# lpiccinelli-eth/UniDepth

Hardware: AMD Instinct MI355X
Metric: images/sec (whole node) + p50 latency, ViT-L/14 518x518 bs=8 (higher is better)
Workload: dtype f16; 1 GPU; UniDepthV2 vitl14 infer(), 518x518, bs=8 per GPU, all 7 outputs on device; value = 2 independent infer() calls in flight per GPU (HIP streams); value_one_call / p50_latency_ms = one call at a time; global_batch=8, parallelism=dp1, inflight=2

## Files before the change

### unidepth_amd/csrc/gemm.hip

```cpp
#include "ud_common.h"

#ifdef UD_TRACE
__device__ unsigned long long* ud_trace_ptr = nullptr;
#define UD_STAMP(slot)                                                                           \
  do {                                                                                           \
    if (ud_trace_ptr && threadIdx.x == 0 && trace_tile < 8)                                      \
      ud_trace_ptr[((size_t)blockIdx.x * 8 + trace_tile) * 8 + (slot)] = wall_clock64();         \
  } while (0)
#else
#define UD_STAMP(slot)
#endif

namespace {

constexpr int UD_LNC_TILES = 2;
constexpr int UD_LNC_PLANE = UD_LNC_TILES * 256;

template <int BN_, int WM_, int WN_>
struct Cfg {
  static constexpr int BM = 128, BN = BN_, BK = 64, WM = WM_, WN = WN_;
  static constexpr int NWM = BM / WM, NWN = BN / WN;
  static constexpr int TM = WM / 16, TN = WN / 16;
  static constexpr int A_BYTES = BM * BK * 2;
  static constexpr int B_BYTES = BN * BK * 2;
// ... 561 lines not shown

template <class C, int EPI, int AMODE, int NST = 2, bool SPLIT = false>
__global__ __launch_bounds__(256) void gemm_kernel(const UdGemm p) {
  extern __shared__ __attribute__((aligned(16))) char smem[];
  const int tiles_n = (p.N + C::BN - 1) / C::BN;
  const int tiles_m = (p.M + C::BM - 1) / C::BM;
  const int nblk = tiles_m * tiles_n;
  int bid = blockIdx.x;
  if constexpr (SPLIT) {
    const int tile_m = (bid >> 1) / tiles_n, tile_n = (bid >> 1) - tile_m * tiles_n;
    gemm_body<C, EPI, AMODE, true, NST, true>(p, smem, tile_m * C::BM, tile_n * C::BN, (const half_t*)p.A, (const half_t*)p.W, p.bias,
                                              (char*)p.out, (char*)p.out2, p.w2, p.b2, p.post_add, bid >> 1, bid & 1);
    return;
  }
  {
    const int q = nblk >> 3, r = nblk & 7;
    const int xcd = bid & 7, idx = bid >> 3;
    bid = (xcd < r ? xcd * (q + 1) : r * (q + 1) + (xcd - r) * q) + idx;
  }
  const int tile_m = bid / tiles_n;
  const int tile_n = bid - tile_m * tiles_n;
  const int m0 = tile_m * C::BM, n0 = tile_n * C::BN;
  const int g = blockIdx.z;
  const half_t* A = (const half_t*)p.A + (long long)g * p.gA;
  const half_t* W = (const half_t*)p.W + (long long)g * p.gW;
  const float* bias = p.bias ? p.bias + (long long)g * p.gBias : nullptr;
  char* out = (char*)p.out + (long long)g * p.gOut * ((EPI == UD_EPI_F16 || EPI == UD_EPI_QKV) ? 2 : 4);
  char* out2 = p.out2 ? (char*)p.out2 + (long long)g * p.gOut2 * 2 : nullptr;
  const float* w2 = p.w2 ? p.w2 + (long long)g * p.gW2 : nullptr;
  const float b2 = g == 0 ? p.b2 : p.b2_g1;
  const float post_add = g == 0 ? p.post_add : p.post_add_g1;
  if constexpr (EPI == UD_EPI_QKV) {
    if (n0 >= p.vsplit) {
      gemm_body<C, EPI, AMODE, false, NST, false>(p, smem, m0, n0, A, W, bias, out, out2, w2, b2, post_add);
      return;
    }
  }
  gemm_body<C, EPI, AMODE, true, NST, false>(p, smem, m0, n0, A, W, bias, out, out2, w2, b2, post_add);
}

template <int MH>
struct BigCfg {
  static constexpr int BM = 64 * MH;
  static constexpr int A_BYTES = BM * 128;
  static constexpr int STAGE = A_BYTES + 32768;
  static constexpr int A_LOADS = BM / 64;
};

template <bool B> struct BoolTag { static constexpr bool value = B; };
constexpr int LNC_TILES = UD_LNC_TILES;
constexpr int LNC_LDS = 2 * UD_LNC_PLANE * 4;

__device__ __forceinline__ void ud_pair16(unsigned& a, unsigned& b) {
  const auto r = __builtin_amdgcn_permlane16_swap(a, b, false, false);
  a = r[0];
  b = r[1];
}
__device__ __forceinline__ void ud_pair32(unsigned& a, unsigned& b) {
  const auto r = __builtin_amdgcn_permlane32_swap(a, b, false, false);
  a = r[0];
  b = r[1];
}
__device__ __forceinline__ unsigned ud_pack2(float x, float y) {
  f32x2 v; v[0] = x; v[1] = y;
  const half2v h = __builtin_convertvector(v, half2v);
  return __builtin_bit_cast(unsigned, h);
}
typedef __attribute__((ext_vector_type(4))) unsigned u32x4;

template <int R, int M>
__device__ __forceinline__ void ud_interleave_reads() {
  constexpr int q = M / (R + 1);
  if constexpr (R >= 1) { __builtin_amdgcn_sched_group_barrier(0x8, q, 0); __builtin_amdgcn_sched_group_barrier(0x100, 1, 0); }
  if constexpr (R >= 2) { __builtin_amdgcn_sched_group_barrier(0x8, q, 0); __builtin_amdgcn_sched_group_barrier(0x100, 1, 0); }
  if constexpr (R >= 3) { __builtin_amdgcn_sched_group_barrier(0x8, q, 0); __builtin_amdgcn_sched_group_barrier(0x100, 1, 0); }
  if constexpr (R >= 4) { __builtin_amdgcn_sched_group_barrier(0x8, q, 0); __builtin_amdgcn_sched_group_barrier(0x100, 1, 0); }
  if constexpr (R >= 5) { __builtin_amdgcn_sched_group_barrier(0x8, q, 0); __builtin_amdgcn_sched_group_barrier(0x100, 1, 0); }
  if constexpr (R >= 6) { __builtin_amdgcn_sched_group_barrier(0x8, q, 0); __builtin_amdgcn_sched_group_barrier(0x100, 1, 0); }
  if constexpr (R >= 7) { __builtin_amdgcn_sched_group_barrier(0x8, q, 0); __builtin_amdgcn_sched_group_barrier(0x100, 1, 0); }
  if constexpr (R >= 8) { __builtin_amdgcn_sched_group_barrier(0x8, q, 0); __builtin_amdgcn_sched_group_barrier(0x100, 1, 0); }
  __builtin_amdgcn_sched_group_barrier(0x8, M - q * R, 0);
}

template <int MH, int EPI, int AMODE, bool BAL = false, bool LNC = false, bool GRP = false, bool W3 = false, bool SPK = false>
__global__ __launch_bounds__(512) void gemm256_kernel(const UdGemm p) {
  extern __shared__ __attribute__((aligned(16))) char smem[];
  using C = BigCfg<MH>;
  static_assert(!W3 || (AMODE == UD_A_DENSE && !BAL && !GRP), "W3: dense A, tile list");
  static_assert(!SPK || (!BAL && !LNC && !GRP && !W3 && (EPI == UD_EPI_F16 || EPI == UD_EPI_F32)), "K split: plain tile list, fp16 / fp32 epilogues");
  constexpr int RING_BYTES = W3 ? 2 * C::A_BYTES + 3 * 32768 : 2 * C::STAGE;
  static_assert(!LNC || (AMODE == UD_A_DENSE && (EPI == UD_EPI_F16 || EPI == UD_EPI_QKV)), "LayerNorm-folded consumer: dense A, fp16 outputs");
  constexpr int BM = C::BM;
  constexpr int TM = 2 * MH;
  const int tid = threadIdx.x;
  const int lane = tid & 63;
  const int wv = __builtin_amdgcn_readfirstlane(tid >> 6);
  const int wm = wv >> 2, wn = wv & 3;
  const int nk = SPK ? (p.K >> 7) : (p.K >> 6);
  const int kbase = SPK ? (int)(blockIdx.x & 1) * nk : 0;
  const int tiles_n = (p.N + 255) >> 8;
  const int tiles_m = (p.M + BM - 1) / BM;
  const int nblk = tiles_m * tiles_n;
  const half_t* A = (const half_t*)p.A;
  const half_t* W = (const half_t*)p.W;

  auto decode = [&](int t, int& m0, int& n0) {
    const int q = nblk >> 3, r = nblk & 7;
    const int xcd = t & 7, idx = t >> 3;
    const int bid = (xcd < r ? xcd * (q + 1) : r * (q + 1) + (xcd - r) * q) + idx;
    const int GM = nblk <= 256 ? 1 : 8;
    const int gsz = GM * tiles_n;
    const int grp = bid / gsz;
    const int first_m = grp * GM;
    const int gm = (tiles_m - first_m) < GM ? (tiles_m - first_m) : GM;
    const int rem = bid - grp * gsz;
    m0 = (first_m + rem % gm) * BM;
    n0 = (rem / gm) << 8;
  };

  const int lrow = tid >> 3;
  const int csrc = (tid & 7) ^ ((lrow >> 1) & 7);
  const ud_rsrc_t rA = ud_make_rsrc(A, 0x80000000u);
  const ud_rsrc_t rW = ud_make_rsrc(W, 0x80000000u);
  unsigned pa[C::A_LOADS];
  unsigned cyx[C::A_LOADS];
  unsigned pb[4];
  const float inv_cc = (AMODE != UD_A_DENSE) ? 1.0f / (float)(p.Cin >> 3) : 0.0f;
  auto setupA = [&](int m0, int mh) {
    int grp = 0;
    if constexpr (GRP) grp = m0 / p.grp_rows;
#pragma unroll
    for (int i = 0; i < C::A_LOADS; ++i) {
      if (i >= mh) continue;
      int m = m0 + lrow + 64 * i;
      m = m < p.M ? m : p.M - 1;
      if constexpr (GRP) {
        if (p.gA == 0) m -= grp * p.grp_rows;
      }
      if constexpr (AMODE == UD_A_DENSE) {
        pa[i] = ((unsigned)m * (unsigned)p.lda + csrc * 8) * 2u;
      } else {
        const int img = m / p.rows_img;
        const int pp = m - img * p.rows_img;
        const int y = pp / p.Wimg;
        pa[i] = (unsigned)((long long)img * p.img_stride) * 2u;
        cyx[i] = pp < p.Himg * p.Wimg ? ((unsigned)y << 16) | (unsigned)(pp - y * p.Wimg) : 0x40000000u;
      }
    }
  };
  auto setupB = [&](int m0, int n0) {
    int grp = 0;
    if constexpr (GRP) grp = m0 / p.grp_rows;
#pragma unroll
    for (int i = 0; i < 4; ++i) {
      int n = n0 + lrow + 64 * i;
      n = n < p.N ? n : p.N - 1;
      pb[i] = ((unsigned)n * (unsigned)p.ldw + csrc * 8) * 2u;
      if constexpr (GRP) pb[i] += (unsigned)grp * (unsigned)p.gW * 2u;
    }
  };
  auto setup = [&](int m0, int n0, int mh) {
    setupA(m0, mh);
    setupB(m0, n0);
  };
  const int a_wt = p.a_wrap > 0 ? (AMODE == UD_A_DENSE ? p.a_wrap >> 6 : p.a_wrap) : 0x7fffffff;
  const int w_wt = p.w_wrap > 0 ? p.w_wrap >> 6 : 0x7fffffff;
  auto a_stage = [&](int stg) -> char* { return smem + stg * (W3 ? C::A_BYTES : C::STAGE); };
  auto b_stage = [&](int stg) -> char* { return W3 ? smem + 2 * C::A_BYTES + stg * 32768 : smem + stg * C::STAGE + C::A_BYTES; };
  auto issueA = [&](int kt, int stg, int mh) {
    char* sb = a_stage(stg) + wv * 1024;
    kt += kbase;
// ... 14 lines not shown
      for (int i = 0; i < C::A_LOADS; ++i) {
        if (i >= mh) continue;
        const int yy = (int)(cyx[i] >> 16) + dy, xx = (int)(cyx[i] & 0xffff) + dx;
        const bool ok = tap < 9 && (unsigned)yy < (unsigned)p.Himg && (unsigned)xx < (unsigned)p.Wimg;
        const unsigned off = ok ? pa[i] + (unsigned)((yy * p.Wimg + xx) * p.cstride + p.coff + cch) * 2u : 0xfffffff0u;
        ud_bufl16(rA, off, 0, sb + i * 8192);
      }
    }
  };
  auto issueB = [&](int kt, int stg) {
    char* sb = b_stage(stg) + wv * 1024;
    kt += kbase;
    const int kb = kt >= w_wt ? kt - w_wt : kt;
#pragma unroll
    for (int i = 0; i < 4; ++i) ud_bufl16(rW, pb[i], kb * 128, sb + i * 8192);
  };
  auto issue = [&](int kt, int stg, int mh) {
    issueA(kt, stg, mh);
    issueB(kt, stg);
  };

  const int fswz = (lane & 15) >> 1;
  const int c0 = ((lane >> 4) ^ fswz) << 4;
  const int c1 = ((4 + (lane >> 4)) ^ fswz) << 4;
  const int b_off = (wn * 64 + (lane & 15)) * 128;

  f32x4 acc[TM][4];
  half8 a0[MH], a1[MH], b0[4], b1[4];
  int stg = 0;
  int stgb = 0;

  constexpr bool ACC_EPI = (EPI == UD_EPI_F32);

  float* const lds_rstd = (float*)(smem + RING_BYTES);
  float* const lds_nm = lds_rstd + UD_LNC_PLANE;
  int tl = 0;

  int m0, n0, mhc = MH;
  int t = SPK ? (int)(blockIdx.x >> 1) : (int)blockIdx.x;
  int bal_k = 0, bal_tb = 0, bal_te = 0, bal_u0 = 0, bal_n0 = 0;
  if constexpr (BAL) {
    const int G = gridDim.x;
    const int cpc = G / tiles_n;
    const int U = (p.M + 63) >> 6;
    int col, r;
    if ((G & 7) == 0 && (cpc & 3) == 0 && (tiles_n & 1) == 0) {
      const int x = blockIdx.x & 7, j = blockIdx.x >> 3;
      const int cx = tiles_n >> 1, rx = cpc >> 2;
      col = (x & 1) * cx + j % cx;
      r = (x >> 1) * rx + j / cx;
    } else if (tiles_n == 1 && (G & 7) == 0) {
      col = 0;
      r = (blockIdx.x & 7) * (G >> 3) + (blockIdx.x >> 3);
    } else {
      const int lc = blockIdx.x;
      col = lc / cpc;
      r = lc - col * cpc;
    }
    const int base = U / cpc, extra = U - base * cpc;
    const int un = base + (r < extra ? 1 : 0);
    if (un == 0) return;
    bal_u0 = r * base + (r < extra ? r : extra);
    bal_k = (un + 3) >> 2;
    bal_tb = un / bal_k;
    bal_te = un - bal_tb * bal_k;
    bal_n0 = col << 8;
    t = 0;
  }
  auto tile_at = [&](int i, int& tm0, int& tn0, int& tmh) {
    if constexpr (BAL) {
      tmh = bal_tb + (i < bal_te ? 1 : 0);
      tm0 = (bal_u0 + i * bal_tb + (i < bal_te ? i : bal_te)) << 6;
      tn0 = bal_n0;
    } else {
      decode(i, tm0, tn0);
      tmh = MH;
    }
  };
  const int tcount = BAL ? bal_k : nblk;
  const int tstep = BAL ? 1 : (SPK ? nblk : (int)gridDim.x);
  tile_at(t, m0, n0, mhc);
  setup(m0, n0, mhc);
  issue(0, 0, mhc);
  if constexpr (W3) issueB(1, 1);
  const ud_rsrc_t rS = ud_make_rsrc(LNC ? p.row_stats_in : nullptr, (unsigned)p.M * 8u);
  auto stats_dma = [&](int tm0, int tmh, int buf) {
    if (wv < 4 && wv < tmh) {
      int m = tm0 + wv * 64 + lane;
      m = m < p.M ? m : p.M - 1;
      ud_bufl4(rS, (unsigned)m * 8u, 0, lds_rstd + buf * 256 + wv * 64);
      ud_bufl4(rS, (unsigned)m * 8u + 4u, 0, lds_nm + buf * 256 + wv * 64);
    }
  };
  if constexpr (LNC) stats_dma(m0, mhc, 0);

  int trace_tile = 0;
  bool first = true;
  for (; t < tcount; t += tstep, ++trace_tile) {
    UD_STAMP(0);
    const int tn = t + tstep;
    const bool has_next = tn < tcount;
    int m0n = 0, n0n = 0, mhn = MH;
    if (has_next) tile_at(tn, m0n, n0n, mhn);
    const bool swap = !(EPI == UD_EPI_QKV && n0 >= p.vsplit);
    auto tile_body = [&](auto MHT) {
    constexpr int MHC = decltype(MHT)::value;
    constexpr int TMC = 2 * MHC;
    constexpr int BMC = 64 * MHC;
    const int a_off = (wm * (BMC / 2) + (lane & 15)) * 128;
    const int mbase = m0 + wm * (BMC / 2), nbase = n0 + wn * 64;

#pragma unroll
    for (int i = 0; i < TMC; ++i)
#pragma unroll
      for (int j = 0; j < 4; ++j) acc[i][j] = (f32x4){0.f, 0.f, 0.f, 0.f};

    bool counted = false;
    if constexpr (ACC_EPI) {
      if (p.accumulate && kbase == 0) {
        int ln = lane;
        asm volatile("" : "+v"(ln));
        if (first && (m0 + BMC <= p.M) && (n0 + 256 <= p.N) && p.rows_in == 0) {
          const float* ob = (const float*)p.out + (size_t)(mbase + (ln & 15)) * p.ldc + nbase + 4 * (ln >> 4);
#pragma unroll
          for (int i = 0; i < TMC; ++i)
#pragma unroll
            for (int j = 0; j < 4; ++j) acc[i][j] = *(const f32x4*)(ob + (size_t)(i * 16) * p.ldc + j * 16);
          counted = true;
        } else {
          gemm_preload_acc<TMC, 4>(p, acc, mbase, nbase, ln, (const char*)p.out);
        }
      }
    }
    if (first) {
      if (counted) asm volatile("s_waitcnt vmcnt(%0)" ::"i"(TMC * 4) : "memory");
      else asm volatile("s_waitcnt vmcnt(0)" ::: "memory");
      __builtin_amdgcn_s_barrier();
      asm volatile("" ::: "memory");
      first = false;
    }
    {
      const char* sa0 = a_stage(stg);
      const char* sb0 = b_stage(W3 ? stgb : stg);
#pragma unroll
      for (int i = 0; i < MHC; ++i) a0[i] = *(const half8*)(sa0 + a_off + i * 2048 + c0);
#pragma unroll
      for (int j = 0; j < 4; ++j) b0[j] = *(const half8*)(sb0 + b_off + j * 2048 + c0);
    }

    auto ktile = [&](auto SW, auto LASTT, int kt, auto PHT) {
      constexpr bool SWAP = decltype(SW)::value;
      constexpr bool LAST = decltype(LASTT)::value;
      constexpr int PH = decltype(PHT)::value;
      const int stgb1 = stgb == 2 ? 0 : stgb + 1, stgb2 = stgb == 0 ? 2 : stgb - 1;
      const char* sa = a_stage(stg);
      const char* sb = b_stage(W3 ? stgb : stg);
      const char* san = a_stage(stg ^ 1);
      const char* sbn = b_stage(W3 ? stgb1 : stg ^ 1);
#define UD_MFMA_HALF(ROW0, AF, BF)                                                                               \
  _Pragma("unroll") for (int i = 0; i < MHC; ++i) _Pragma("unroll") for (int j = 0; j < 4; ++j) {               \
    if constexpr (SWAP) acc[ROW0 + i][j] = __builtin_amdgcn_mfma_f32_16x16x32_f16(BF[j], AF[i], acc[ROW0 + i][j], 0, 0, 0); \
    else acc[ROW0 + i][j] = __builtin_amdgcn_mfma_f32_16x16x32_f16(AF[i], BF[j], acc[ROW0 + i][j], 0, 0, 0);   \
  }
      if constexpr (W3) {
        if constexpr (PH == 2) {
          if (has_next) {
            if constexpr (LNC) stats_dma(m0n, mhn, (tl + 1) & 1);
            setupA(m0n, mhn);
            issueA(0, stg ^ 1, mhn);
            issueB(1, stgb2);
          }
        } else if constexpr (PH == 1) {
          issueA(kt + 1, stg ^ 1, MHC);
          if (has_next) {
            setupB(m0n, n0n);
            issueB(0, stgb2);
          }
        } else {
          issueA(kt + 1, stg ^ 1, MHC);
          issueB(kt + 2, stgb2);
        }
      } else if constexpr (LAST) {
        if (has_next) {
          setup(m0n, n0n, mhn);
          issue(0, stg ^ 1, mhn);
          if constexpr (LNC) stats_dma(m0n, mhn, (tl + 1) & 1);
        }
      } else {
        issue(kt + 1, stg ^ 1, MHC);
      }
#pragma unroll
      for (int i = 0; i < MHC; ++i) a1[i] = *(const half8*)(sa + a_off + (MHC + i) * 2048 + c0);
      UD_MFMA_HALF(0, a0, b0)
      ud_interleave_reads<MHC, 4 * MHC>();
      __builtin_amdgcn_sched_barrier(0);
#pragma unroll
      for (int i = 0; i < MHC; ++i) a0[i] = *(const half8*)(sa + a_off + i * 2048 + c1);
#pragma unroll
      for (int j = 0; j < 4; ++j) b1[j] = *(const half8*)(sb + b_off + j * 2048 + c1);
      UD_MFMA_HALF(MHC, a1, b0)
      ud_interleave_reads<MHC + 4, 4 * MHC>();
      __builtin_amdgcn_sched_barrier(0);
#pragma unroll
      for (int i = 0; i < MHC; ++i) a1[i] = *(const half8*)(sa + a_off + (MHC + i) * 2048 + c1);
      UD_MFMA_HALF(0, a0, b1)
      ud_interleave_reads<MHC, 4 * MHC>();
      __builtin_amdgcn_sched_barrier(0);
      if constexpr (W3) {
        if (PH == 0 || has_next) asm volatile("s_waitcnt vmcnt(4)\n\ts_waitcnt lgkmcnt(0)" ::: "memory");
        else asm volatile("s_waitcnt vmcnt(0)\n\ts_waitcnt lgkmcnt(0)" ::: "memory");
      } else {
        asm volatile("s_waitcnt vmcnt(0)\n\ts_waitcnt lgkmcnt(0)" ::: "memory");
      }
      __builtin_amdgcn_s_barrier();
      asm volatile("" ::: "memory");
      if constexpr (!LAST) {
#pragma unroll
        for (int i = 0; i < MHC; ++i) a0[i] = *(const half8*)(san + a_off + i * 2048 + c0);
#pragma unroll
        for (int j = 0; j < 4; ++j) b0[j] = *(const half8*)(sbn + b_off + j * 2048 + c0);
      }
      UD_MFMA_HALF(MHC, a1, b1)
      if constexpr (!LAST) ud_interleave_reads<MHC + 4, 4 * MHC>();
      __builtin_amdgcn_sched_barrier(0);
#undef UD_MFMA_HALF
      stg ^= 1;
      if constexpr (W3) stgb = stgb1;
    };

    auto kloop = [&](auto SW) {
      if constexpr (W3) {
        for (int kt = 0; kt < nk - 2; ++kt) ktile(SW, BoolTag<false>{}, kt, IntTag<0>{});
        ktile(SW, BoolTag<false>{}, nk - 2, IntTag<1>{});
        ktile(SW, BoolTag<true>{}, nk - 1, IntTag<2>{});
      } else {
        for (int kt = 0; kt < nk - 1; ++kt) ktile(SW, BoolTag<false>{}, kt, IntTag<0>{});
        ktile(SW, BoolTag<true>{}, nk - 1, IntTag<0>{});
      }
    };
    UD_STAMP(1);
    if constexpr (EPI == UD_EPI_QKV) {
      if (swap) kloop(BoolTag<true>{});
      else kloop(BoolTag<false>{});
    } else {
      kloop(BoolTag<true>{});
    }
    UD_STAMP(2);
    if constexpr (SPK) {
      constexpr int NQ = TMC * 4;
      const int half = (int)(blockIdx.x & 1);
      f32x4* mine = (f32x4*)p.splitk_ws + ((size_t)(t * 2 + half) * 8 + wv) * (NQ * 64) + lane;
      const f32x4* other = (const f32x4*)p.splitk_ws + ((size_t)(t * 2 + (half ^ 1)) * 8 + wv) * (NQ * 64) + lane;
#pragma unroll
      for (int i = 0; i < TMC; ++i)
#pragma unroll
        for (int j = 0; j < 4; ++j) {
          const f32x4 v = acc[i][j];
          asm volatile("global_store_dwordx4 %0, %1, off sc0 sc1\n\ts_nop 2" ::"v"(mine + (i * 4 + j) * 64), "v"(v) : "memory");
        }
      asm volatile("s_waitcnt vmcnt(0)" ::: "memory");
      __builtin_amdgcn_s_barrier();
      unsigned* tk = (unsigned*)(smem + RING_BYTES);
      if (tid == 0) *tk = atomicAdd((unsigned*)p.splitk_cnt + t, 1u);
      asm volatile("s_waitcnt lgkmcnt(0)" ::: "memory");
      __builtin_amdgcn_s_barrier();
      const unsigned ticket = *tk;
      if ((ticket & 1u) == 0) return;
#pragma unroll
      for (int c = 0; c < NQ / 8; ++c) {
        f32x4 o[8];
#pragma unroll
        for (int q = 0; q < 8; ++q) asm volatile("global_load_dwordx4 %0, %1, off sc0 sc1" : "=v"(o[q]) : "v"(other + (c * 8 + q) * 64) : "memory");
        asm volatile("s_waitcnt vmcnt(0)" : "+v"(o[0]), "+v"(o[1]), "+v"(o[2]), "+v"(o[3]), "+v"(o[4]), "+v"(o[5]), "+v"(o[6]), "+v"(o[7])::"memory");
#pragma unroll
        for (int q = 0; q < 8; ++q) acc[(c * 8 + q) >> 2][(c * 8 + q) & 3] += o[q];
      }
    }
    const float* const lnst = LNC ? lds_rstd + (tl & 1) * 256 + wm * (BMC / 2) : nullptr;

    const float* biasp = p.bias;
    if constexpr (GRP) {
      if (p.bias) biasp = p.bias + (long long)(m0 / p.grp_rows) * p.gBias;
    }
    const bool full = (m0 + BMC <= p.M) && (n0 + 256 <= p.N) && p.rows_in == 0 && p.add == nullptr && p.bias != nullptr;
    bool fast = false;
    bool ticket_taken = false;
    unsigned ticket_val = 0;
    int eln = lane;
    asm volatile("" : "+v"(eln));
    const int frow = eln & 15, fq = eln >> 4;
    if constexpr (EPI == UD_EPI_F16 || EPI == UD_EPI_QKV) {
      if (swap) {
        fast = full && (p.ldc & 7) == 0;
        if (fast) {
          const int act = p.act;
          f32x4 bv[4], ws[4];
#pragma unroll
          for (int j = 0; j < 4; ++j) bv[j] = *(const f32x4*)(biasp + nbase + j * 16 + 4 * fq);
          if constexpr (LNC) {
#pragma unroll
            for (int j = 0; j < 4; ++j) ws[j] = *(const f32x4*)(p.wsum + nbase + j * 16 + 4 * fq);
          }
          half_t* o = (half_t*)p.out + (size_t)(mbase + frow) * p.ldc + nbase + 16 * (fq & 1) + 8 * (fq >> 1);
          auto body = [&](auto ACT) {
            constexpr int AC = decltype(ACT)::value;
#pragma unroll
            for (int i = 0; i < TMC; ++i) {
              unsigned w[4][2];
              float rs = 0.f, nmr = 0.f;
              if constexpr (LNC) {
                rs = lnst[i * 16 + frow];
                nmr = lnst[UD_LNC_PLANE + i * 16 + frow];
              }
#pragma unroll
// ... 541 lines not shown
        const int hy = hp / 18, hx = hp - hy * 18;
        int iy = cur.y0 - 1 + hy, ix = cur.x0 - 1 + hx;
        iy = iy < 0 ? -iy : (iy >= p.Himg ? 2 * p.Himg - 2 - iy : iy);
        ix = ix < 0 ? -ix : (ix >= p.Wimg ? 2 * p.Wimg - 2 - ix : ix);
        const bool ok = hp < 324 && iy >= cur.ylo && iy <= cur.yhi && ix >= cur.xlo && ix <= cur.xhi;
        half8 o8;
#pragma unroll
        for (int e = 0; e < 8; ++e) o8[e] = (half_t)0.f;
        if (ok) {
          const float fy = ups_sy * (float)iy, fx = ups_sx * (float)ix;
          const int sy0 = (int)fy, sx0 = (int)fx;
          const int sy1 = sy0 + (sy0 < p.Hsrc - 1), sx1 = sx0 + (sx0 < p.Wsrc - 1);
          const half_t ly = (half_t)(fy - (float)sy0), lx = (half_t)(fx - (float)sx0);
          const int cs = (cpos ^ ((hp >> 1) & 7)) << 4;
          const half8 h00 = *(const half8*)(patch + ((sy0 - cur.syA) * cur.PC + (sx0 - cur.sxA)) * 128 + cs);
          const half8 h01 = *(const half8*)(patch + ((sy0 - cur.syA) * cur.PC + (sx1 - cur.sxA)) * 128 + cs);
          const half8 h10 = *(const half8*)(patch + ((sy1 - cur.syA) * cur.PC + (sx0 - cur.sxA)) * 128 + cs);
          const half8 h11 = *(const half8*)(patch + ((sy1 - cur.syA) * cur.PC + (sx1 - cur.sxA)) * 128 + cs);
          const half8 top = h00 + lx * (h01 - h00);
          const half8 bot = h10 + lx * (h11 - h10);
          o8 = top + ly * (bot - top);
        }
        *(half8*)(halo + i * 1024 + lane * 16) = o8;
      }
    }
    __syncthreads();
    const int tn = t + (int)gridDim.x;
    Geo nxt = cur;
    if (tn < tiles_g) {
      nxt = geo(tn);
      issue_patch(nxt);
    }
    f32x4 acc[4][2];
#pragma unroll
    for (int i = 0; i < 4; ++i)
#pragma unroll
      for (int j = 0; j < 2; ++j) acc[i][j] = (f32x4){0.f, 0.f, 0.f, 0.f};
#pragma unroll
    for (int tap = 0; tap < 9; ++tap) {
      const int dy = tap / 3, dx = tap - dy * 3;
#pragma unroll
      for (int ks = 0; ks < 2; ++ks) {
        half8 af[4];
#pragma unroll
        for (int i = 0; i < 4; ++i) {
          const int hp = (wv * 4 + i + dy) * 18 + px + dx;
          af[i] = *(const half8*)(halo + hp * 128 + (((ks * 4 + fq) ^ ((hp >> 1) & 7)) << 4));
        }
#pragma unroll
        for (int i = 0; i < 4; ++i)
#pragma unroll
          for (int j = 0; j < 2; ++j) acc[i][j] = __builtin_amdgcn_mfma_f32_16x16x32_f16(bfr[tap][ks][j], af[i], acc[i][j], 0, 0, 0);
        __builtin_amdgcn_sched_barrier(0);
      }
    }
    f32x4 bv[2], wv2[2];
#pragma unroll
    for (int j = 0; j < 2; ++j) {
      bv[j] = *(const f32x4*)(bias + j * 16 + 4 * fq);
      wv2[j] = *(const f32x4*)(w2 + j * 16 + 4 * fq);
    }
#pragma unroll
    for (int i = 0; i < 4; ++i) {
      const int y = cur.y0 + wv * 4 + i, x = cur.x0 + px;
      const bool ok = y < p.Himg && x < p.Wimg;
      const size_t row = ((size_t)cur.b * p.Himg + y) * p.Wimg + x;
      float part = 0.f;
#pragma unroll
      for (int j = 0; j < 2; ++j)
#pragma unroll
        for (int r = 0; r < 4; ++r) part += ud_lrelu(acc[i][j][r] + bv[j][r]) * wv2[j][r];
      part += __shfl_xor(part, 16, 64);
      part += __shfl_xor(part, 32, 64);
      if (ok && fq == 0) {
        float yv = part + (g == 0 ? p.b2 : p.b2_g1);
        yv = fminf(fmaxf(yv, -8.0f), 8.0f);
        ((float*)p.out)[(long long)g * p.gOut + row] = __expf(yv + (g == 0 ? p.post_add : p.post_add_g1));
      }
    }
    cur = nxt;
  }
}

constexpr size_t SPK_SLOT_BYTES = (size_t)192 * 256 * 4;
constexpr int UPS_PATCH = 13;

enum Sched {
  S_TILE128,
  S_RING,
  S_LIST,
  S_BALANCED,
  S_LIST_SPLITK,
  S_PINGPONG,
  S_DUO,
  S_CONV_TILE,
  S_HEAD_REGW
};

struct Route {
  Sched sched;
  bool large;
  int bn;
  bool splitk;
  int mh;
  bool lnc;
  bool grp;
  bool w3;
  int nt;
  int prio;
  UdGemm merged;
};

inline bool big_split_ok(const UdGemm& d) {
  if (d.amode != UD_A_DENSE && d.amode != UD_A_CONV3_ZERO) return false;
  if (d.epi != UD_EPI_F16 && d.epi != UD_EPI_F32) return false;
  if (d.groups > 1 || d.row_stats_in || d.row_stats_out || d.max_out || d.a_wrap || d.w_wrap || (d.K & 127) || d.K < 2048) return false;
  const int tiles = ((d.N + 255) >> 8) * ((d.M + 191) / 192);
  if (tiles > 128 || tiles < 32 || d.M < 1024 || d.N < 192) return false;
  if (!d.splitk_ws || !d.splitk_cnt || (size_t)d.splitk_ws_bytes < 2 * (size_t)tiles * SPK_SLOT_BYTES) return false;
  return true;
}

inline int bal_cpc(const UdGemm& d) {
  const int tiles_n = (d.N + 255) >> 8;
  if (tiles_n > 128 || (d.N & 255)) return 0;
  const int cpc = 256 / tiles_n;
  const int U = (d.M + 63) >> 6;
  return (U / cpc >= 2) ? cpc : 0;
}
inline double bal_time(const UdGemm& d, int cpc) {
  const int U = (d.M + 63) >> 6;
  const int un = (U + cpc - 1) / cpc;
  const int k = (un + 3) >> 2;
  return 8.0 + (un * (30.0 / 4.0) + (k - 1) * 2.5) * ((double)d.K / 1024.0);
}

inline int pick_tiles(const UdGemm& d) {
  if (d.amode == UD_A_CONV3_REFLECT || d.groups > 1 || d.M < 1024 || d.N < 192 || (d.K & 63)) return UD_PICK_TILE128;
  if (d.amode != UD_A_DENSE && d.rows_img <= 0) return UD_PICK_TILE128;
  if (d.amode == UD_A_CONV3_ZERO && d.epi != UD_EPI_F16 && d.epi != UD_EPI_F32) return UD_PICK_TILE128;
  {
    const double a_bytes = d.amode == UD_A_DENSE ? 2.0 * d.M * d.lda : 2.0 * ((double)(d.M / d.rows_img) + 1.0) * (double)d.img_stride;
    if (a_bytes >= 2147483648.0 || 2.0 * d.N * d.ldw >= 2147483648.0) return UD_PICK_TILE128;
  }
  if (d.epi == UD_EPI_QKV && (d.vsplit & 255)) return UD_PICK_TILE128;
  const int cpc = bal_cpc(d);
  const bool bal_ok = (d.amode == UD_A_DENSE || (d.amode == UD_A_CONV3_ZERO && d.epi != UD_EPI_QKV)) &&
                      (d.epi == UD_EPI_F16 || d.epi == UD_EPI_F32 || d.epi == UD_EPI_QKV) && cpc > 0;
  switch (d.tile_hint) {
    case UD_HINT_TILE128: case UD_HINT_PLAIN128: case UD_HINT_RING: case UD_HINT_RING_SPLITK: return UD_PICK_TILE128;
    case UD_HINT_LIST256: return UD_PICK_LIST256;
    case UD_HINT_LIST192: case UD_HINT_LIST192_W2: return UD_PICK_LIST192;
    case UD_HINT_LIST192_SPLITK: return big_split_ok(d) ? UD_PICK_LIST192_SPLITK : UD_PICK_TILE128;
    case UD_HINT_PINGPONG: case UD_HINT_DUO_FIRST: case UD_HINT_DUO_EQUAL: case UD_HINT_DUO_SECOND:
      return UD_PICK_LIST192;
    case UD_HINT_BALANCED: if (bal_ok) return UD_PICK_BALANCED; break;
    default: if (d.tile_hint > UD_HINT_DUO_SECOND) return UD_PICK_TILE128; break;
  }
  const double kk = (double)d.K / 1024.0;
  const double tn = (double)((d.N + 255) / 256);
  const double t256 = 8.0 + ceil(tn * ((d.M + 255) / 256) / 256.0) * 30.0 * kk;
  const double t192 = 8.0 + ceil(tn * ((d.M + 191) / 192) / 256.0) * 23.5 * kk;
  const double tbal = (bal_ok && ((d.M + 63) / 64 + cpc - 1) / cpc > 4) ? bal_time(d, cpc) : 1e30;
  const double small_tiles = (double)((d.N + 127) / 128) * ((d.M + 127) / 128);
  const double t_small = 6.0 + ceil(small_tiles / 256.0) * 0.5 * 21.5 * kk;
  double t_big = t256 <= t192 ? t256 : t192;
// ... 86 lines not shown
    }
  }
  if (r.large) {
    r.lnc = d.row_stats_in != nullptr;
    if (bt == UD_PICK_LIST192_SPLITK) {
      r.sched = S_LIST_SPLITK;
    } else if (bt == UD_PICK_BALANCED && !d.row_stats_final) {
      r.sched = S_BALANCED;
    } else {
      r.sched = S_LIST;
      r.mh = bt == UD_PICK_LIST256 ? 4 : 3;
      r.w3 = r.mh == 3 && d.amode == UD_A_DENSE && d.K >= 128 && d.tile_hint != UD_HINT_LIST192_W2;
    }
    return r;
  }
  const int ring = d.N > 64 && d.epi != UD_EPI_D2S ? ring_variant(d, ud_debug_flags_host()) : 0;
  if (ring) {
    r.sched = S_RING;
    r.splitk = ring == 2;
    return r;
  }
  r.sched = S_TILE128;
  r.bn = d.N > 64 ? 128 : d.N > 32 ? 64 : 32;
  return r;
}

int pick_code(const Route& r) {
  switch (r.sched) {
    case S_TILE128: return r.bn == 128 ? UD_PICK_TILE128 : r.bn == 64 ? UD_PICK_TILE128_BN64 : UD_PICK_TILE128_BN32;
    case S_RING: return r.splitk ? UD_PICK_RING_SPLITK : UD_PICK_RING;
    case S_LIST: return (r.mh == 3 ? UD_PICK_LIST192 : UD_PICK_LIST256) + (r.lnc ? UD_PICK_LN_CONSUMER : 0) + (r.grp ? UD_PICK_GROUPED : 0);
    case S_BALANCED: return UD_PICK_BALANCED + (r.lnc ? UD_PICK_LN_CONSUMER : 0);
    case S_LIST_SPLITK: return UD_PICK_LIST192_SPLITK;
    case S_PINGPONG: return UD_PICK_PINGPONG;
    case S_DUO: return UD_PICK_DUO;
    case S_CONV_TILE: case S_HEAD_REGW: return UD_PICK_CONV_TILE;
  }
  return -1;
}

int kernel_name(const Route& r, const UdGemm& d, char* buf, int cap) {
  const auto b = [](bool v) { return v ? "true" : "false"; };
  int n = -1;
  switch (r.sched) {
    case S_TILE128:
      n = snprintf(buf, cap, "gemm_kernel<Cfg<%s>, %d, %d, 2, false>", r.bn == 128 ? "128, 64, 64" : r.bn == 64 ? "64, 64, 32" : "32, 32, 32", d.epi, d.amode);
      break;
    case S_RING: n = snprintf(buf, cap, "gemm_kernel<Cfg<128, 64, 64>, %d, %d, 4, %s>", d.epi, d.amode, b(r.splitk)); break;
    case S_LIST: n = snprintf(buf, cap, "gemm256_kernel<%d, %d, %d, false, %s, %s, %s, false>", r.mh, d.epi, d.amode, b(r.lnc), b(r.grp), b(r.w3)); break;
    case S_BALANCED: n = snprintf(buf, cap, "gemm256_kernel<4, %d, %d, true, %s, false, false, false>", d.epi, d.amode, b(r.lnc)); break;
    case S_LIST_SPLITK: n = snprintf(buf, cap, "gemm256_kernel<3, %d, %d, false, false, false, false, true>", d.epi, d.amode); break;
    case S_PINGPONG: n = snprintf(buf, cap, "gemm_pp_f32_kernel<3, 8>"); break;
    case S_DUO: n = snprintf(buf, cap, "gemm_pp_f32_kernel<3, 4>"); break;
    case S_CONV_TILE:
      n = snprintf(buf, cap, "conv_tile_kernel<%d, %d, %s, %s>", r.nt, d.epi, b(d.amode >= UD_A_CONV3_REFLECT), b(d.amode == UD_A_CONV3_REFLECT_UP));
      break;
    case S_HEAD_REGW: n = snprintf(buf, cap, "conv_head_regw_kernel"); break;
  }
  return n >= 0 && n < cap ? UD_OK : UD_ERR_BAD_ARG;
}

constexpr bool is_dense_f16_f32_qkv(int epi, int amode) { return amode == UD_A_DENSE && (epi == UD_EPI_F16 || epi == UD_EPI_F32 || epi == UD_EPI_QKV); }
constexpr bool has_large_tile(int epi, int amode) {
  return amode == UD_A_DENSE ? epi != UD_EPI_HEAD : amode == UD_A_CONV3_ZERO && (epi == UD_EPI_F16 || epi == UD_EPI_F32);
}
constexpr bool has_ln_consumer(int epi, int amode) { return amode == UD_A_DENSE && (epi == UD_EPI_F16 || epi == UD_EPI_QKV); }

template <class C, int EPI, int AMODE, int NST = 2, bool SPLIT = false>
int launch128(const UdGemm& d, hipStream_t s) {
  constexpr bool plain = EPI == UD_EPI_F16   ? AMODE <= UD_A_CONV3_REFLECT
                         : EPI == UD_EPI_F32 ? AMODE <= UD_A_CONV3_ZERO
                         : EPI == UD_EPI_QKV ? AMODE == UD_A_DENSE && C::BN == 128
                         : EPI == UD_EPI_D2S ? AMODE == UD_A_DENSE
                                             : AMODE == UD_A_CONV3_REFLECT && C::BN == 32;
  if constexpr (NST == 2 ? plain : C::BN == 128 && is_dense_f16_f32_qkv(EPI, AMODE) && !(SPLIT && EPI == UD_EPI_QKV)) {
    const int tiles = ((d.N + C::BN - 1) / C::BN) * ((d.M + C::BM - 1) / C::BM);
    const dim3 grid((SPLIT ? 2 : 1) * tiles, 1, d.groups > 0 ? d.groups : 1);
    return ud_launch_lds<gemm_kernel<C, EPI, AMODE, NST, SPLIT>>(
        grid, dim3(256), NST * C::STAGE_BYTES, s, NST == 2 ? "ud_gemm_f16 launch" : SPLIT ? "ud_gemm_f16 (4-stage ring, K split) launch" : "ud_gemm_f16 (4-stage ring) launch", d);
  }
  return UD_ERR_UNSUPPORTED;
}

template <int MH, int EPI, int AMODE, bool LNC, bool GRP, bool W3>
int launch256(const UdGemm& d, hipStream_t s) {
  if constexpr (has_large_tile(EPI, AMODE) && (!LNC || (has_ln_consumer(EPI, AMODE) && !GRP)) && (!GRP || (MH == 4 && is_dense_f16_f32_qkv(EPI, AMODE))) &&
                (!W3 || (MH == 3 && AMODE == UD_A_DENSE && !GRP))) {
    const int tiles = ((d.N + 255) >> 8) * ((d.M + BigCfg<MH>::BM - 1) / BigCfg<MH>::BM);
    const int lds = (W3 ? 2 * BigCfg<MH>::A_BYTES + 3 * 32768 : 2 * BigCfg<MH>::STAGE) + (LNC ? LNC_LDS : 0) + (EPI == UD_EPI_F32 ? 64 : 0);
    return ud_launch_lds<gemm256_kernel<MH, EPI, AMODE, false, LNC, GRP, W3>>(
        dim3(tiles < 256 ? tiles : 256), dim3(512), lds, s, W3 ? "ud_gemm_f16 (large tile, 3-deep weight ring) launch" : "ud_gemm_f16 (large tile) launch", d);
  }
  return UD_ERR_UNSUPPORTED;
}

template <int EPI, int AMODE, bool LNC>
int launch256bal(const UdGemm& d, hipStream_t s) {
  if constexpr (has_large_tile(EPI, AMODE) && EPI != UD_EPI_D2S && (!LNC || has_ln_consumer(EPI, AMODE))) {
    const int tiles_n = (d.N + 255) >> 8;
    return ud_launch_lds<gemm256_kernel<4, EPI, AMODE, true, LNC>>(dim3(bal_cpc(d) * tiles_n), dim3(512), 2 * BigCfg<4>::STAGE + (LNC ? LNC_LDS : 0), s,
                                                                   "ud_gemm_f16 (large tile, row-balanced) launch", d);
  }
  return UD_ERR_UNSUPPORTED;
}

template <int EPI, int AMODE>
int launch256sk(const UdGemm& d, hipStream_t s) {
  if constexpr (has_large_tile(EPI, AMODE) && (EPI == UD_EPI_F16 || EPI == UD_EPI_F32)) {
    const int tiles = ((d.N + 255) >> 8) * ((d.M + 191) / 192);
    return ud_launch_lds<gemm256_kernel<3, EPI, AMODE, false, false, false, false, true>>(dim3(2 * tiles), dim3(512), 2 * BigCfg<3>::STAGE + 64, s,
                                                                                          "ud_gemm_f16 (large tile, K split) launch", d);
  }
  return UD_ERR_UNSUPPORTED;
}

constexpr int UPS_LDS = (UPS_PATCH * UPS_PATCH * 128 + 1023) / 1024 * 1024;
template <int NT, int EPI, int AMODE>
int launch_conv_tile(const UdGemm& d, hipStream_t s) {
  constexpr bool REFLECT = AMODE >= UD_A_CONV3_REFLECT, UPS = AMODE == UD_A_CONV3_REFLECT_UP;
  if constexpr (EPI == UD_EPI_HEAD ? NT == 2 && REFLECT : EPI == UD_EPI_F16 && (AMODE == UD_A_CONV3_ZERO || AMODE == UD_A_CONV3_REFLECT)) {
    const dim3 grid(((d.Wimg + 15) >> 4) * ((d.Himg + 15) >> 4), d.M / d.rows_img, d.groups > 0 ? d.groups : 1);
    return ud_launch_lds<conv_tile_kernel<NT, EPI, REFLECT, UPS>>(grid, dim3(256), HALO_BYTES + 2 * NT * 16 * 128 + (UPS ? UPS_LDS : 0), s,
                                                                  "ud_gemm_f16 (halo-tile conv) launch", d);
  }
  return UD_ERR_UNSUPPORTED;
}

int launch_head_regw(const UdGemm& d, hipStream_t s) {
  const int B = d.M / d.rows_img;
  const int tiles_x = (d.Wimg + 15) >> 4, tiles_img = tiles_x * ((d.Himg + 15) >> 4), tiles_g = tiles_img * B;
  const int G = d.groups > 0 ? d.groups : 1;
  int wgs = (512 + G - 1) / G;
  wgs = wgs < tiles_g ? wgs : tiles_g;
  return ud_launch_lds<conv_head_regw_kernel>(dim3(wgs, G), dim3(256), HALO_BYTES + UPS_LDS, s, "ud_gemm_f16 (head conv, register-resident weights) launch", d, tiles_x,
                                              tiles_img, tiles_g);
}

template <class F>
int with_epi_amode(const UdGemm& d, F f) {
  const auto with_amode = [&](auto epi) {
    switch (d.amode) {
      case UD_A_DENSE: return f(epi, IntTag<UD_A_DENSE>{});
      case UD_A_CONV3_ZERO: return f(epi, IntTag<UD_A_CONV3_ZERO>{});
      case UD_A_CONV3_REFLECT: return f(epi, IntTag<UD_A_CONV3_REFLECT>{});
      case UD_A_CONV3_REFLECT_UP: return f(epi, IntTag<UD_A_CONV3_REFLECT_UP>{});
    }
    return (int)UD_ERR_UNSUPPORTED;
  };
  switch (d.epi) {
    case UD_EPI_F16: return with_amode(IntTag<UD_EPI_F16>{});
    case UD_EPI_F32: return with_amode(IntTag<UD_EPI_F32>{});
    case UD_EPI_QKV: return with_amode(IntTag<UD_EPI_QKV>{});
    case UD_EPI_D2S: return with_amode(IntTag<UD_EPI_D2S>{});
    case UD_EPI_HEAD: return with_amode(IntTag<UD_EPI_HEAD>{});
  }
  return (int)UD_ERR_UNSUPPORTED;
}

int launch_route(const Route& r, const UdGemm& desc, hipStream_t s) {
  const UdGemm& d = r.grp ? r.merged : desc;
  const int rc = with_epi_amode(d, [&](auto epi, auto amode) -> int {
    constexpr int EPI = decltype(epi)::value, AMODE = decltype(amode)::value;
    switch (r.sched) {
      case S_TILE128:
        return r.bn == 128  ? launch128<Cfg<128, 64, 64>, EPI, AMODE>(d, s)
               : r.bn == 64 ? launch128<Cfg<64, 64, 32>, EPI, AMODE>(d, s)
                            : launch128<Cfg<32, 32, 32>, EPI, AMODE>(d, s);
      case S_RING: return r.splitk ? launch128<Cfg<128, 64, 64>, EPI, AMODE, 4, true>(d, s) : launch128<Cfg<128, 64, 64>, EPI, AMODE, 4>(d, s);
      case S_LIST:
        if (r.grp) return launch256<4, EPI, AMODE, false, true, false>(d, s);
        if (r.mh == 4) return r.lnc ? launch256<4, EPI, AMODE, true, false, false>(d, s) : launch256<4, EPI, AMODE, false, false, false>(d, s);
        if (r.w3) return r.lnc ? launch256<3, EPI, AMODE, true, false, true>(d, s) : launch256<3, EPI, AMODE, false, false, true>(d, s);
        return r.lnc ? launch256<3, EPI, AMODE, true, false, false>(d, s) : launch256<3, EPI, AMODE, false, false, false>(d, s);
      case S_BALANCED: return r.lnc ? launch256bal<EPI, AMODE, true>(d, s) : launch256bal<EPI, AMODE, false>(d, s);
      case S_LIST_SPLITK: return launch256sk<EPI, AMODE>(d, s);
      case S_PINGPONG: return ud_gemm_pp_launch(d, s);
      case S_DUO: return ud_gemm_duo_launch(d, s, r.prio);
      case S_CONV_TILE: return r.nt == 4 ? launch_conv_tile<4, EPI, AMODE>(d, s) : launch_conv_tile<2, EPI, AMODE>(d, s);
      case S_HEAD_REGW: return launch_head_regw(d, s);
    }
    return UD_ERR_UNSUPPORTED;
  });
// ... 23 lines not shown
    return UD_ERR_BAD_ARG;
  }
  if (d.row_stats_in) {
    if (d.amode != UD_A_DENSE || (d.epi != UD_EPI_F16 && d.epi != UD_EPI_QKV) || !d.wsum || d.add || d.rows_in || (d.N & 15) || !large) {
      ud_set_error("ud_gemm_f16: LayerNorm-folded consumer (row_stats_in) needs dense A, an fp16 epilogue without add / row remap, wsum, N % 16 == 0 "
                   "and a problem the large-tile kernel takes (ud_gemm_pick >= 3)");
      return UD_ERR_UNSUPPORTED;
    }
  }
  if (d.max_out && (d.epi != UD_EPI_F32 || d.rows_in || d.accumulate == 2)) {
    ud_set_error("ud_gemm_f16: max_out needs the fp32 epilogue without a row remap");
    return UD_ERR_UNSUPPORTED;
  }
  if (d.row_stats_out) {
    if (d.epi != UD_EPI_F32 || (d.N & 63) || (!large && (d.N <= 64 || d.groups > 1))) {
      ud_set_error("ud_gemm_f16: row_stats_out needs the fp32 epilogue, N % 64 == 0 and 64-column wave tiles (N > 64, no groups)");
      return UD_ERR_UNSUPPORTED;
    }
    if (d.row_stats_final && (!large || !d.row_stats_ticket || d.ln_D <= 0 || d.N > 1024 || (d.N & 127) || d.groups > 1)) {
      ud_set_error("ud_gemm_f16: row_stats_final (in-kernel reduction of the row statistics) needs the large-tile kernel, a ticket buffer, ln_D, "
                   "N <= 1024 and N % 128 == 0 (the finalizer reads the 64-column slabs in pairs)");
      return UD_ERR_UNSUPPORTED;
    }
  } else if (d.row_stats_final) {
    ud_set_error("ud_gemm_f16: row_stats_final without row_stats_out");
    return UD_ERR_BAD_ARG;
  }
  if (d.amode == UD_A_CONV3_REFLECT_UP && d.epi != UD_EPI_HEAD) {
    ud_set_error("ud_gemm_f16: CONV3_REFLECT_UP is implemented for the HEAD epilogue only");
    return UD_ERR_UNSUPPORTED;
  }
  if (d.amode != UD_A_DENSE && (!d.zeros || (d.Cin & 7) || d.K < 9 * d.Cin || d.rows_img < d.Himg * d.Wimg)) {
    ud_set_error("ud_gemm_f16: bad conv geometry");
    return UD_ERR_BAD_ARG;
  }
  if (d.epi == UD_EPI_QKV && (d.amode != UD_A_DENSE || !d.out2 || (d.vsplit % 128) || (d.tok_per_img & 3) || (d.kv_ld & 3) || d.N <= 64)) {
    ud_set_error("ud_gemm_f16: bad QKV epilogue geometry");
    return UD_ERR_BAD_ARG;
  }
  if (d.up_src && d.epi != UD_EPI_D2S && d.epi != UD_EPI_QKV) {
    ud_set_error("ud_gemm_f16: up_src belongs to the D2S epilogue");
    return UD_ERR_BAD_ARG;
  }
  if (d.epi == UD_EPI_D2S) {
    if (d.amode != UD_A_DENSE || (d.d2s_Co & 3)) {
      ud_set_error("ud_gemm_f16: bad D2S epilogue geometry");
      return UD_ERR_BAD_ARG;
    }
    if (d.up_src && (d.up_H < 1 || d.up_W < 1 || 2 * d.up_H != d.d2s_Hin * d.d2s_k || 2 * d.up_W != d.d2s_Win * d.d2s_k || (d.up_ld & 3) || d.up_ld < d.d2s_Co ||
                     d.up_img_rows < d.up_H * d.up_W || d.groups > 1)) {
      ud_set_error("ud_gemm_f16: up_src (fused x2 up-sampling under the D2S accumulate) needs 2 * up_H == d2s_Hin * d2s_k (same for W), up_ld % 4 == 0, "
                   "up_ld >= d2s_Co, up_img_rows >= up_H * up_W");
      return UD_ERR_BAD_ARG;
    }
  }
  if (d.epi == UD_EPI_HEAD) {
    if ((d.amode != UD_A_CONV3_REFLECT && d.amode != UD_A_CONV3_REFLECT_UP) || d.N != 32 || !d.w2 || !d.bias) {
      ud_set_error("ud_gemm_f16: HEAD epilogue needs reflect conv, N == 32");
      return UD_ERR_BAD_ARG;
    }
    if (d.amode == UD_A_CONV3_REFLECT_UP) {
      const bool fits = 17.0 * (d.Hsrc - 1) / (d.Himg > 1 ? d.Himg - 1 : 1) + 3.0 <= UPS_PATCH && 17.0 * (d.Wsrc - 1) / (d.Wimg > 1 ? d.Wimg - 1 : 1) + 3.0 <= UPS_PATCH;
      if (!halo || d.Hsrc < 1 || d.Wsrc < 1 || (d.cstride & 7) || !fits) {
        ud_set_error("ud_gemm_f16: CONV3_REFLECT_UP needs Cin % 64 == 0, dense images, Hsrc / Wsrc >= 1 and an up-sampling factor >= ~1.7");
        return UD_ERR_BAD_ARG;
      }
    }
  }
  return launch_route(r, d, (hipStream_t)stream);
}

#ifdef UD_TRACE
extern "C" int ud_trace_set(void* buf) {
  return hipMemcpyToSymbol(HIP_SYMBOL(ud_trace_ptr), &buf, sizeof(buf)) == hipSuccess ? UD_OK : UD_ERR_LAUNCH;
}
#endif

extern "C" int ud_gemm_pick(const UdGemm* desc) { return pick_code(route(*desc)); }

extern "C" int ud_gemm_kernel_name(const UdGemm* desc, char* buf, int cap) {
  if (!desc || !buf || cap <= 0) return UD_ERR_BAD_ARG;
  return kernel_name(route(*desc), *desc, buf, cap);
}
```

Measured before the change: 630.2 images/s.

## Add staggered ping-pong K loop for large-tile LayerNorm-folded GEMMs

```diff
diff --git a/unidepth_amd/csrc/gemm.hip b/unidepth_amd/csrc/gemm.hip
--- a/unidepth_amd/csrc/gemm.hip
+++ b/unidepth_amd/csrc/gemm.hip
@@ -667,11 +667,22 @@
   __builtin_amdgcn_sched_group_barrier(0x8, M - q * R, 0);
 }
 
-template <int MH, int EPI, int AMODE, bool BAL = false, bool LNC = false, bool GRP = false, bool W3 = false, bool SPK = false>
+constexpr int UD_WAIT_VM4_LGKM0 = 0x0074;
+constexpr int UD_WAIT_VM0_LGKM0 = 0x0070;
+constexpr int UD_WAIT_VM0 = 0x0F70;
+#define UD_STG_BAR()                         \
+  do {                                       \
+    __builtin_amdgcn_sched_barrier(0);       \
+    __builtin_amdgcn_s_barrier();            \
+    __builtin_amdgcn_sched_barrier(0);       \
+  } while (0)
+
+template <int MH, int EPI, int AMODE, bool BAL = false, bool LNC = false, bool GRP = false, bool W3 = false, bool SPK = false, bool STG = false>
 __global__ __launch_bounds__(512) void gemm256_kernel(const UdGemm p) {
   extern __shared__ __attribute__((aligned(16))) char smem[];
   using C = BigCfg<MH>;
   static_assert(!W3 || (AMODE == UD_A_DENSE && !BAL && !GRP), "W3: dense A, tile list");
+  static_assert(!STG || (!W3 && !GRP && !SPK), "staggered loop: two [A | W] buffers, plain tile list or row-balanced spans");
   static_assert(!SPK || (!BAL && !LNC && !GRP && !W3 && (EPI == UD_EPI_F16 || EPI == UD_EPI_F32)), "K split: plain tile list, fp16 / fp32 epilogues");
   constexpr int RING_BYTES = W3 ? 2 * C::A_BYTES + 3 * 32768 : 2 * C::STAGE;
   static_assert(!LNC || (AMODE == UD_A_DENSE && (EPI == UD_EPI_F16 || EPI == UD_EPI_QKV)), "LayerNorm-folded consumer: dense A, fp16 outputs");
@@ -852,7 +863,7 @@
   tile_at(t, m0, n0, mhc);
   setup(m0, n0, mhc);
   issue(0, 0, mhc);
-  if constexpr (W3) issueB(1, 1);
+  if constexpr (W3 || STG) issueB(1, 1);
   const ud_rsrc_t rS = ud_make_rsrc(LNC ? p.row_stats_in : nullptr, (unsigned)p.M * 8u);
   auto stats_dma = [&](int tm0, int tmh, int buf) {
     if (wv < 4 && wv < tmh) {
@@ -904,12 +915,13 @@
     }
     if (first) {
       if (counted) asm volatile("s_waitcnt vmcnt(%0)" ::"i"(TMC * 4) : "memory");
+      else if constexpr (STG) __builtin_amdgcn_s_waitcnt(UD_WAIT_VM0);
       else asm volatile("s_waitcnt vmcnt(0)" ::: "memory");
       __builtin_amdgcn_s_barrier();
       asm volatile("" ::: "memory");
       first = false;
     }
-    {
+    if constexpr (!STG) {
       const char* sa0 = a_stage(stg);
       const char* sb0 = b_stage(W3 ? stgb : stg);
 #pragma unroll
@@ -998,8 +1010,87 @@
       if constexpr (W3) stgb = stgb1;
     };
 
+    auto sktile = [&](auto SW, auto PHT, int kt) {
+      constexpr bool SWAP = decltype(SW)::value;
+      constexpr int PH = decltype(PHT)::value;
+      const char* sa = a_stage(stg);
+      const char* sb = b_stage(stg);
+#define UD_STG_QUAD(ROW0, JH)                                                                                                     \
+  _Pragma("unroll") for (int ks = 0; ks < 2; ++ks) _Pragma("unroll") for (int i = 0; i < MHC; ++i)                                \
+      _Pragma("unroll") for (int j = 2 * (JH); j < 2 * (JH) + 2; ++j) {                                                           \
+    if constexpr (SWAP) acc[ROW0 + i][j] = __builtin_amdgcn_mfma_f32_16x16x32_f16(ks ? b1[j] : b0[j], ks ? a1[i] : a0[i], acc[ROW0 + i][j], 0, 0, 0); \
+    else acc[ROW0 + i][j] = __builtin_amdgcn_mfma_f32_16x16x32_f16(ks ? a1[i] : a0[i], ks ? b1[j] : b0[j], acc[ROW0 + i][j], 0, 0, 0);                \
+  }
+#pragma unroll
+      for (int j = 0; j < 4; ++j) {
+        b0[j] = *(const half8*)(sb + b_off + j * 2048 + c0);
+        b1[j] = *(const half8*)(sb + b_off + j * 2048 + c1);
+      }
+#pragma unroll
+      for (int i = 0; i < MHC; ++i) {
+        a0[i] = *(const half8*)(sa + a_off + i * 2048 + c0);
+        a1[i] = *(const half8*)(sa + a_off + i * 2048 + c1);
+      }
+      if constexpr (PH == 2) {
+        if (has_next) {
+          if constexpr (LNC) stats_dma(m0n, mhn, (tl + 1) & 1);
+          setupA(m0n, mhn);
+          issueA(0, stg ^ 1, mhn);
+        }
+      } else {
+        issueA(kt + 1, stg ^ 1, MHC);
+      }
+      asm volatile("s_waitcnt lgkmcnt(0)" : "+v"(b0[0]), "+v"(b0[1]), "+v"(b0[2]), "+v"(b0[3]), "+v"(b1[0]), "+v"(b1[1]), "+v"(b1[2]), "+v"(b1[3])::"memory");
+      UD_STG_BAR();
+      UD_STG_QUAD(0, 0)
+      UD_STG_QUAD(0, 1)
+      UD_STG_BAR();
+#pragma unroll
+      for (int i = 0; i < MHC; ++i) {
+        a0[i] = *(const half8*)(sa + a_off + (MHC + i) * 2048 + c0);
+        a1[i] = *(const half8*)(sa + a_off + (MHC + i) * 2048 + c1);
+      }
+#define UD_STG_WAIT(IMM)                   \
+  do {                                     \
+    asm volatile("" ::: "memory");         \
+    __builtin_amdgcn_s_waitcnt(IMM);       \
+    asm volatile("" ::: "memory");         \
+  } while (0)
+      if constexpr (PH == 0) {
+        issueB(kt + 2, stg);
+        UD_STG_WAIT(UD_WAIT_VM4_LGKM0);
+      } else {
+        if (has_next) {
+          if constexpr (PH == 1) {
+            setupB(m0n, n0n);
+            issueB(0, stg);
+          } else {
+            issueB(1, stg);
+          }
+          UD_STG_WAIT(UD_WAIT_VM4_LGKM0);
+        } else {
+          UD_STG_WAIT(UD_WAIT_VM0_LGKM0);
+        }
+      }
+#undef UD_STG_WAIT
+      UD_STG_BAR();
+      UD_STG_QUAD(MHC, 1)
+      UD_STG_QUAD(MHC, 0)
+      UD_STG_BAR();
+#undef UD_STG_QUAD
+      stg ^= 1;
+    };
+
     auto kloop = [&](auto SW) {
-      if constexpr (W3) {
+      if constexpr (STG) {
+        if (wm == 1) UD_STG_BAR();
+        constexpr int KT0 = (!BAL || MHC == 2) ? 1 : 0;
+        if constexpr (KT0) sktile(SW, IntTag<0>{}, 0);
+        for (int kt = KT0; kt < nk - 2; ++kt) sktile(SW, IntTag<0>{}, kt);
+        sktile(SW, IntTag<1>{}, nk - 2);
+        sktile(SW, IntTag<2>{}, nk - 1);
+        if (wm == 0) UD_STG_BAR();
+      } else if constexpr (W3) {
         for (int kt = 0; kt < nk - 2; ++kt) ktile(SW, BoolTag<false>{}, kt, IntTag<0>{});
         ktile(SW, BoolTag<false>{}, nk - 2, IntTag<1>{});
         ktile(SW, BoolTag<true>{}, nk - 1, IntTag<2>{});
@@ -1707,6 +1798,12 @@
   }
 }
 
+#ifdef UD_GEMM256_CODEGEN
+template __global__ void gemm256_kernel<3, UD_EPI_QKV, UD_A_DENSE, false, true, false, false, false, true>(const UdGemm);
+template __global__ void gemm256_kernel<4, UD_EPI_F16, UD_A_DENSE, true, true, false, false, false, true>(const UdGemm);
+}
+#else
+
 constexpr size_t SPK_SLOT_BYTES = (size_t)192 * 256 * 4;
 constexpr int UPS_PATCH = 13;
 
@@ -1959,11 +2056,19 @@
   return UD_ERR_UNSUPPORTED;
 }
 
+constexpr bool stg_list(int mh, int epi, int amode, bool lnc, bool w3) { return mh == 3 && epi == UD_EPI_QKV && amode == UD_A_DENSE && lnc && w3; }
+constexpr bool stg_balanced(int epi, int amode, bool lnc) { return epi == UD_EPI_F16 && amode == UD_A_DENSE && lnc; }
+
 template <int MH, int EPI, int AMODE, bool LNC, bool GRP, bool W3>
 int launch256(const UdGemm& d, hipStream_t s) {
   if constexpr (has_large_tile(EPI, AMODE) && (!LNC || (has_ln_consumer(EPI, AMODE) && !GRP)) && (!GRP || (MH == 4 && is_dense_f16_f32_qkv(EPI, AMODE))) &&
                 (!W3 || (MH == 3 && AMODE == UD_A_DENSE && !GRP))) {
     const int tiles = ((d.N + 255) >> 8) * ((d.M + BigCfg<MH>::BM - 1) / BigCfg<MH>::BM);
+    if constexpr (stg_list(MH, EPI, AMODE, LNC, W3)) {
+      if (d.K >= 256)
+        return ud_launch_lds<gemm256_kernel<MH, EPI, AMODE, false, LNC, false, false, false, true>>(
+            dim3(tiles < 256 ? tiles : 256), dim3(512), 2 * BigCfg<MH>::STAGE + LNC_LDS, s, "ud_gemm_f16 (large tile, staggered loop) launch", d);
+    }
     const int lds = (W3 ? 2 * BigCfg<MH>::A_BYTES + 3 * 32768 : 2 * BigCfg<MH>::STAGE) + (LNC ? LNC_LDS : 0) + (EPI == UD_EPI_F32 ? 64 : 0);
     return ud_launch_lds<gemm256_kernel<MH, EPI, AMODE, false, LNC, GRP, W3>>(
         dim3(tiles < 256 ? tiles : 256), dim3(512), lds, s, W3 ? "ud_gemm_f16 (large tile, 3-deep weight ring) launch" : "ud_gemm_f16 (large tile) launch", d);
@@ -1975,6 +2080,11 @@
 int launch256bal(const UdGemm& d, hipStream_t s) {
   if constexpr (has_large_tile(EPI, AMODE) && EPI != UD_EPI_D2S && (!LNC || has_ln_consumer(EPI, AMODE))) {
     const int tiles_n = (d.N + 255) >> 8;
+    if constexpr (stg_balanced(EPI, AMODE, LNC)) {
+      if (d.K >= 256)
+        return ud_launch_lds<gemm256_kernel<4, EPI, AMODE, true, LNC, false, false, false, true>>(
+            dim3(bal_cpc(d) * tiles_n), dim3(512), 2 * BigCfg<4>::STAGE + LNC_LDS, s, "ud_gemm_f16 (large tile, row-balanced, staggered loop) launch", d);
+    }
     return ud_launch_lds<gemm256_kernel<4, EPI, AMODE, true, LNC>>(dim3(bal_cpc(d) * tiles_n), dim3(512), 2 * BigCfg<4>::STAGE + (LNC ? LNC_LDS : 0), s,
                                                                    "ud_gemm_f16 (large tile, row-balanced) launch", d);
   }
@@ -2164,3 +2274,4 @@
   if (!desc || !buf || cap <= 0) return UD_ERR_BAD_ARG;
   return kernel_name(route(*desc), *desc, buf, cap);
 }
+#endif
```

Result: no change. 635.8 images/s (median of 6 runs) (+0.9%).
